# YamaneKoyo/mri-to-speech

Measured on AMD Instinct MI355X. Metric: rtMRI frames/s end-to-end (256x256 frames -> 64-bin mel -> 11413 Hz wav), higher is better.
Workload: dtype bf16x3; 1 GPU; e2e rtMRI->wav, 64 clips x 30 frames per GPU at 256x256 (configs[3] per-GPU share); clips_per_gpu=64, frames_per_clip=30, global_batch_clips=64, hw=256, parallelism=dp1, chunk=1920

## Files before the change

mri-to-speech_amd/csrc/er_sp_fused.hip:

```cpp
#include <algorithm>

#include "kernels.hpp"
#include "prof.hpp"

namespace m2s {
namespace {

__device__ __attribute__((aligned(16))) uint4 g_ersp_zero[4];

__device__ __forceinline__ void dma16(const void* src, void* lds_wave_base) {
  __builtin_amdgcn_global_load_lds(src, lds_wave_base, 16, 0, 0);
}
__device__ __forceinline__ uint32_t lds_off(const void* p) {
  return (uint32_t)(size_t)(const __attribute__((address_space(3))) char*)p;
}
__device__ __forceinline__ uint2 lds_u2(const void* p) {
  uint2 r;
  asm volatile("ds_read_b64 %0, %1\n\ts_waitcnt lgkmcnt(0)" : "=v"(r) : "v"(lds_off(p)));
  return r;
}
__device__ __forceinline__ float4 lds_f4(const void* p) {
  float4 r;
  asm volatile("ds_read_b128 %0, %1\n\ts_waitcnt lgkmcnt(0)" : "=v"(r) : "v"(lds_off(p)));
  return r;
}
template <int N>
__device__ __forceinline__ void wait_vm() {
  asm volatile("s_waitcnt vmcnt(%0)" ::"n"(N) : "memory");
}
__device__ __forceinline__ bf16x8 frag(const char* p) { return *reinterpret_cast<const bf16x8*>(p); }
__device__ __forceinline__ f32x4 mfma(bf16x8 a, bf16x8 b, f32x4 c) {
  return __builtin_amdgcn_mfma_f32_16x16x32_bf16(a, b, c, 0, 0, 0);
}

struct ErSpArgs {
  const bf16_t* x;
  const bf16_t* wst;
  const float* bexp;
  const float* bpwl;
  bf16_t* y;
  int N, H, W, tiles_x, tiles_y;
};

template <int TH, int CSI, int NT, int ON, int NW, int MRG>
__global__ void __launch_bounds__(64 * NW, NW == 4 ? 2 : 1) er_sp_kernel(const ErSpArgs a) {
  constexpr int TW = 16, HW = TW + 2, HH = TH + 2, HPIX = HH * HW;
  constexpr int HPB = (HPIX + 63) / 64;
  constexpr int HPLANE = HPB * 1024;
  constexpr int CH = CSI / 8;
  constexpr int HBUF = 2 * CH * HPLANE;
  constexpr int HP = 2 * CH * HPB / NW;
  static_assert((2 * CH * HPB) % NW == 0, "halo pieces must divide over the waves");
  constexpr int PPW = (MRG * NT + NW - 1) / NW;
  constexpr int SLOT = PPW * NW * 1024;
  constexpr int KC = CSI / 32, NCE = 9 * KC * 2;
  constexpr int MID = NT * 16, KS = MID / 32, PN = ON * KS;
  constexpr int NPS = (PN + NT - 1) / NT;
  constexpr int NST = (NCE + 2 * NPS) / MRG;
  static_assert(MRG == 1 || (MRG == 2 && NPS == 1 && NCE % 2 == 0), "merged stages");
  constexpr int RPW = TH / NW;
  constexpr int ST = RPW * ON * 2;
  static_assert(NT % 2 == 0 && ON * 16 == CSI && TH % NW == 0, "er_sp shape");

  extern __shared__ __attribute__((aligned(16))) char smem[];
  char* ring = smem;
  char* hbuf = smem + 3 * SLOT;
  float* bexp_l = reinterpret_cast<float*>(hbuf + 2 * HBUF);
  const int tid = threadIdx.x, lane = tid & 63;
  const int wave = __builtin_amdgcn_readfirstlane(tid >> 6);
  const int g = lane >> 4, r16 = lane & 15;
  const int tpi = a.tiles_x * a.tiles_y, ntiles = a.N * tpi;

  const void* zpage = g_ersp_zero;
  asm volatile("" : "+s"(zpage));
  auto stage_dma = [&](int ls, int slot) {
#pragma unroll
    for (int j = 0; j < PPW; ++j) {
      const int piece = wave * PPW + j;
      const void* src = piece < MRG * NT ? (const void*)(a.wst + ((size_t)(ls * MRG * NT + piece) * 64 + lane) * 8) : zpage;
      dma16(src, ring + slot * SLOT + piece * 1024);
    }
  };
  auto halo_dma = [&](int tile, char* buf) {
    const int n = tile / tpi, tr = tile - n * tpi;
    const int ty0 = (tr / a.tiles_x) * TH - 1, tx0 = (tr - (tr / a.tiles_x) * a.tiles_x) * TW - 1;
    const bf16_t* xi = a.x + (size_t)n * a.H * a.W * (2 * CSI);
#pragma unroll
    for (int j = 0; j < HP; ++j) {
      const int piece = wave * HP + j, pc = piece / HPB, pb = piece - pc * HPB;
      const int p = pb * 64 + lane, hy = p / HW, hx = p - hy * HW;
      const int iy = ty0 + hy, ix = tx0 + hx;
      const void* src = zpage;
      if (p < HPIX && iy >= 0 && iy < a.H && ix >= 0 && ix < a.W)
        src = xi + ((size_t)iy * a.W + ix) * (2 * CSI) + (pc / CH) * CSI + (pc % CH) * 8;
      dma16(src, buf + pc * HPLANE + pb * 1024);
    }
  };

  for (int i = tid; i < MID; i += 64 * NW) bexp_l[i] = a.bexp[i];
  __syncthreads();
  float4 bp[ON];
#pragma unroll
  for (int on = 0; on < ON; ++on) bp[on] = *reinterpret_cast<const float4*>(a.bpwl + on * 16 + 4 * g);

#ifndef ERSP_PRIO
#define ERSP_PRIO 1
#endif
  if (ERSP_PRIO && NW == 8 && wave >= 4) __builtin_amdgcn_s_setprio(1);
  int q = 0;
  if ((int)blockIdx.x < ntiles) {
    stage_dma(0, 0);
    stage_dma(1, 1);
    halo_dma(blockIdx.x, hbuf);
  }
  for (int it = 0, tile = blockIdx.x; tile < ntiles; tile += gridDim.x, ++it) {
    const bool has_next = tile + (int)gridDim.x < ntiles;
    const char* hb = hbuf + (it & 1) * HBUF;
    const int n = tile / tpi, tr = tile - n * tpi;
    const int oy0 = (tr / a.tiles_x) * TH, ox = (tr - (tr / a.tiles_x) * a.tiles_x) * TW + r16;

    auto begin_stage = [&](int ls) -> const char* {
      if (ls == 0) {
        if (it == 0) wait_vm<0>();
        else wait_vm<PPW + ST>();
      } else if (ls == 1) {
        if (has_next) wait_vm<ST + PPW + HP>();
        else wait_vm<ST + PPW>();
      } else if (ls == 2) {
        if (has_next) wait_vm<HP + PPW>();
        else wait_vm<PPW>();
      } else if (ls + 1 < NST || has_next) {
        wait_vm<PPW>();
      } else {
        wait_vm<0>();
      }
      __builtin_amdgcn_s_barrier();
      asm volatile("" ::: "memory");
      if (ls + 2 < NST) stage_dma(ls + 2, (q + 2) % 3);
      else if (has_next) stage_dma(ls + 2 - NST, (q + 2) % 3);
      if (ls == 0 && has_next) halo_dma(tile + gridDim.x, hbuf + ((it + 1) & 1) * HBUF);
      const char* ws = ring + (q % 3) * SLOT + lane * 16;
      ++q;
      return ws;
    };

    f32x4 acc[RPW][NT];
#pragma unroll
    for (int i = 0; i < RPW; ++i)
#pragma unroll
      for (int nt = 0; nt < NT; ++nt) acc[i][nt] = f32x4{0.f, 0.f, 0.f, 0.f};
#pragma unroll 1
    for (int ks = 0; ks < 9 * KC; ++ks) {
      const int t = ks / KC, kc = ks - t * KC, ky = t / 3, kx = t - (t / 3) * 3;
      bf16x8 bh[RPW], bl[RPW];
      const char* wsm = MRG == 2 ? begin_stage(ks) : nullptr;
      {
        const char* ws = MRG == 2 ? wsm : begin_stage(2 * ks);
#pragma unroll
        for (int i = 0; i < RPW; ++i) {
          const int pix = (RPW * wave + i + ky) * HW + r16 + kx;
          bh[i] = frag(hb + (kc * 4 + g) * HPLANE + pix * 16);
          bl[i] = frag(hb + (CH + kc * 4 + g) * HPLANE + pix * 16);
        }
#pragma unroll
        for (int nt = 0; nt < NT; ++nt) {
          const bf16x8 af = frag(ws + nt * 1024);
#pragma unroll
          for (int i = 0; i < RPW; ++i) acc[i][nt] = mfma(af, bl[i], mfma(af, bh[i], acc[i][nt]));
        }
      }
      {
        const char* ws = MRG == 2 ? wsm + NT * 1024 : begin_stage(2 * ks + 1);
#pragma unroll
        for (int nt = 0; nt < NT; ++nt) {
          const bf16x8 af = frag(ws + nt * 1024);
#pragma unroll
          for (int i = 0; i < RPW; ++i) acc[i][nt] = mfma(af, bh[i], acc[i][nt]);
        }
      }
    }

    bf16x8 mh[RPW][KS], ml[RPW][KS];
#pragma unroll
    for (int kk = 0; kk < KS; ++kk)
#pragma unroll
      for (int i = 0; i < RPW; ++i) {
        float v[8];
#pragma unroll
        for (int hh = 0; hh < 2; ++hh) {
          const int nt = 2 * kk + hh;
          const float4 bb = lds_f4(bexp_l + nt * 16 + 4 * g);
          v[4 * hh + 0] = silu(acc[i][nt][0] + bb.x);
          v[4 * hh + 1] = silu(acc[i][nt][1] + bb.y);
          v[4 * hh + 2] = silu(acc[i][nt][2] + bb.z);
          v[4 * hh + 3] = silu(acc[i][nt][3] + bb.w);
// ... 7 lines not shown

    f32x4 o[RPW][ON];
#pragma unroll
    for (int i = 0; i < RPW; ++i)
#pragma unroll
      for (int on = 0; on < ON; ++on) o[i][on] = f32x4{0.f, 0.f, 0.f, 0.f};
    const char* wpm = MRG == 2 ? begin_stage(NCE / 2) : nullptr;
#pragma unroll
    for (int pl = 0; pl < 2; ++pl)
#pragma unroll
      for (int ps = 0; ps < NPS; ++ps) {
        const char* ws = MRG == 2 ? wpm + pl * NT * 1024 : begin_stage(NCE + pl * NPS + ps);
#pragma unroll
        for (int nt = 0; nt < NT; ++nt) {
          const int j = ps * NT + nt;
          if (j >= PN) break;
          const int kk = j / ON, on = j - (j / ON) * ON;
          const bf16x8 af = frag(ws + nt * 1024);
#pragma unroll
          for (int i = 0; i < RPW; ++i) {
            o[i][on] = mfma(af, mh[i][kk], o[i][on]);
            if (pl == 0) o[i][on] = mfma(af, ml[i][kk], o[i][on]);
          }
        }
      }

#pragma unroll
    for (int i = 0; i < RPW; ++i) {
      const int ry = RPW * wave + i, oy = oy0 + ry;
      const int cpix = ((ry + 1) * HW + r16 + 1) * 16;
#pragma unroll
      for (int on = 0; on < ON; ++on) {
        const int c4 = on * 16 + 4 * g;
        float rh[4], rl[4];
        unpack_bf16x4(lds_u2(hb + (c4 >> 3) * HPLANE + cpix + (c4 & 7) * 2), rh);
        unpack_bf16x4(lds_u2(hb + (CH + (c4 >> 3)) * HPLANE + cpix + (c4 & 7) * 2), rl);
        const float v[4] = {o[i][on][0] + bp[on].x + rh[0] + rl[0], o[i][on][1] + bp[on].y + rh[1] + rl[1],
                            o[i][on][2] + bp[on].z + rh[2] + rl[2], o[i][on][3] + bp[on].w + rh[3] + rl[3]};
        uint2 h, l;
        split4(v, h, l);
        bf16_t* yo = a.y + (((size_t)n * a.H + oy) * a.W + ox) * (2 * CSI) + c4;
        *reinterpret_cast<uint2*>(yo) = h;
        *reinterpret_cast<uint2*>(yo + CSI) = l;
      }
    }
  }
  wait_vm<0>();
}

template <int TH, int CSI, int NT, int ON, int NW, int MRG>
void launch_t(const ErSpArgs& a, const char* name, double flops, double bytes, hipStream_t s) {
  constexpr int HW = 18, HPB = ((TH + 2) * HW + 63) / 64, CH = CSI / 8, PPW = (MRG * NT + NW - 1) / NW;
  const size_t lds = 3 * (size_t)PPW * NW * 1024 + 2 * (size_t)(2 * CH * HPB * 1024) + NT * 16 * sizeof(float);
  M2S_CHECK(lds <= (NW == 4 ? 80 : 160) * 1024, "er_sp: LDS budget");
  allow_lds(reinterpret_cast<const void*>(&er_sp_kernel<TH, CSI, NT, ON, NW, MRG>));
  const int cus = device_cus();
  const int grid = std::min(a.N * a.tiles_x * a.tiles_y, (NW == 4 ? 2 : 1) * cus);
  ProfScope ps(name, flops, bytes, s);
  hipLaunchKernelGGL((er_sp_kernel<TH, CSI, NT, ON, NW, MRG>), dim3(grid), dim3(64 * NW), lds, s, a);
  M2S_HIP(hipGetLastError());
}

int tile_rows(int cs_in) { return cs_in == 32 ? 16 : 8; }

}

bool er_sp_supported(int H, int W, int cs_in, int mid, int cs_out) {
  const bool shape = (cs_in == 32 && mid == 128 && cs_out == 32) || (cs_in == 64 && mid == 224 && cs_out == 64);
  return shape && H > 0 && W > 0 && W % 16 == 0 && H % tile_rows(cs_in) == 0;
}

int er_sp_nt_stages(int cs_in, int mid, int cs_out, int* nt) {
  *nt = mid / 16;
  const int kc = cs_in / 32, pn = (cs_out / 16) * (mid / 32);
  return 9 * kc * 2 + 2 * ((pn + *nt - 1) / *nt);
}

void launch_er_sp(const void* x, int N, int H, int W, int cs_in, int mid, int cs_out, const void* wst, const float* bexp,
                  const float* bpwl, void* y, double flops, double bytes, hipStream_t s, bool merged) {
  M2S_CHECK(er_sp_supported(H, W, cs_in, mid, cs_out) && N > 0, "er_sp: unsupported shape");
  ErSpArgs a;
  a.x = static_cast<const bf16_t*>(x);
  a.wst = static_cast<const bf16_t*>(wst);
  a.bexp = bexp;
  a.bpwl = bpwl;
  a.y = static_cast<bf16_t*>(y);
  a.N = N;
  a.H = H;
  a.W = W;
  a.tiles_x = W / 16;
  a.tiles_y = H / tile_rows(cs_in);
  if (cs_in == 32 && merged)
    launch_t<16, 32, 8, 2, 8, 2>(a, "er_sp_kernel<16, 32, 8, 2, 8, 2>", flops, bytes, s);
  else if (cs_in == 32)
    launch_t<16, 32, 8, 2, 8, 1>(a, "er_sp_kernel<16, 32, 8, 2, 8, 1>", flops, bytes, s);
  else
    launch_t<8, 64, 14, 4, 8, 1>(a, "er_sp_kernel<8, 64, 14, 4, 8, 1>", flops, bytes, s);
}

}
```

mri-to-speech_amd/csrc/kernels.hpp:

```cpp
#pragma once

#include "m2s_common.hpp"

namespace m2s {

enum AsyncCode : unsigned { M2S_ASYNC_LSTM = 1u, M2S_ASYNC_WS = 2u };
struct AsyncReport {
  unsigned spin_max = 1u << 20;
  unsigned* err = nullptr;
};
__device__ __forceinline__ void report_async(unsigned* err, unsigned code, int lane) {
  if (err && lane == 0) __hip_atomic_store(err, code, __ATOMIC_RELAXED, __HIP_MEMORY_SCOPE_SYSTEM);
}

template <typename T>
void launch_stem(const float* frames, int N, int H, int W, int OH, int OW, int pad_t, int pad_l,
                 const float* w9, const float* bias, int cout, int cs_out, T* y, hipStream_t s);

int dw_pixel_blocks(int OH, int OW);
template <typename T>
void launch_dwconv(const T* x, int N, int IH, int IW, int OH, int OW, int stride, int pad_t, int pad_l,
                   int C, int cs, const float* w9, const float* bias, T* y, float* sums, hipStream_t s);

template <typename T>
// ... 50 lines not shown
void launch_rb1_fused(const bf16_t* x, bf16_t* s, int B, int L, int C, int k, int np, const int* dil,
                      const bf16_t* const* w1, const float* const* b1, const bf16_t* const* w2,
                      const float* const* b2, int kp, int accum, float div, bool split, double flops, double bytes,
                      hipStream_t st);

void launch_stem_b0(const float* frames, int N, int H, int W, int OH, int OW, int pad_t, int pad_l, const float* w9,
                    const float* b9, const void* w0, const float* b0, int kp0, const void* w1, const float* b1,
                    int kp1, void* y, bool split, double flops, double bytes, hipStream_t s);

bool se_excite_supported(int rd, int kp2, int cs_mid);
void launch_se_excite(const void* mean, int N, int mid, int cs_mid, const void* w1, int kp1, const float* b1,
                      int rd, const void* w2, int kp2, const float* b2, void* gate, bool split, hipStream_t s);

bool er_fused_supported(int H, int W, int cin, int mid, int cout, int kp_exp, int kp_pwl);
void launch_er_fused(const bf16_t* x, int N, int H, int W, const bf16_t* wexp, const float* bexp, const bf16_t* wpwl,
                     const float* bpwl, bf16_t* y, double flops, double bytes, hipStream_t s);

bool er8_fused_supported(int H, int W, int cin, int mid, int cout);
void launch_er8_fused(const bf16_t* x, int N, int H, int W, const uint8_t* wexp, const float* sexp, const float* bexp,
                      const uint8_t* wpwl, const float* spwl, const float* bpwl, bf16_t* y, double flops, double bytes,
                      hipStream_t s, const uint8_t* x8 = nullptr, uint8_t* y8 = nullptr);

bool er2_fused_supported(int H, int W, int cs_in, int mid, int cout, int kp_exp, int kp_pwl);
int er2_stage_elems();
bool er8w_fused_supported(int H, int W, int cs_in, int mid, int cout);
size_t er8w_stream_bytes();
void launch_er8w_fused(const bf16_t* x, const uint8_t* x8, int N, int H, int W, const uint8_t* wst, const float* sexp,
                       const float* bexp, const float* spwl, const float* bpwl, bf16_t* y, uint8_t* y8, double flops,
                       double bytes, hipStream_t s);
void launch_er2_fused(const bf16_t* x, int N, int H, int W, const bf16_t* wst, const float* bexp, const float* bpwl,
                      bf16_t* y, double flops, double bytes, hipStream_t s);

bool er_sp_supported(int H, int W, int cs_in, int mid, int cs_out);
int er_sp_nt_stages(int cs_in, int mid, int cs_out, int* nt);
void launch_er_sp(const void* x, int N, int H, int W, int cs_in, int mid, int cs_out, const void* wst, const float* bexp,
                  const float* bpwl, void* y, double flops, double bytes, hipStream_t s, bool merged = true);

bool ers2_fused_supported(int OH, int OW, int cs_in, int mid, int cs_out, int kp_exp, int kp_pwl);
int ers2_exp_elems(int cs_in, int mid);
bool ers2_sp_supported(int OH, int OW, int cs_in, int mid, int cs_out);
void launch_ers2_sp(const void* x, int N, int H, int W, int OH, int OW, int pad_t, int pad_l, int cs_in, int mid,
                    int cs_out, const void* wexp, const float* bexp, const void* wpwl, const float* bpwl, void* y,
                    double flops, double bytes, hipStream_t s);
void launch_ers2_fused(const bf16_t* x, int N, int H, int W, int OH, int OW, int pad_t, int pad_l, int cs_in, int mid,
                       int cs_out, const bf16_t* wexp, const float* bexp, const bf16_t* wpwl, const float* bpwl,
                       bf16_t* y, double flops, double bytes, hipStream_t s, uint8_t* y8 = nullptr);

void launch_preprocess(const uint8_t* frames, int N, int H, int W, int channels, float* out, hipStream_t s);

template <typename T>
void launch_gap(const T* x, int N, int P, int C, int cs, float* feats, hipStream_t s);

void launch_lstm_step(const float* pre, const float* whh, float* hs, float* cst, int B, int T, int H,
                      int step, hipStream_t s);

bool lstm_persistent_supported(int H);
size_t lstm_persistent_sync_bytes();
bool lstm_small_supported(int B, int H);
size_t lstm_small_sync_bytes();
void launch_lstm_small(const float* pre, const float* whh, float* hs, int B, int T, int H, void* sync, unsigned spin_max,
                       unsigned* err_host, hipStream_t s, unsigned* epoch = nullptr);
constexpr unsigned LSTM_SPIN_MAX = 1u << 24;
bool lstm_mid_supported(int B, int H);
size_t lstm_mid_sync_bytes();
void launch_lstm_mid(const float* pre, const float* whh, float* hs, int B, int T, int H, void* sync, unsigned spin_max,
                     unsigned* err_host, hipStream_t s);
void launch_lstm_persistent(const float* pre, const float* whh, float* hs, int B, int T, int H, void* sync,
                            unsigned spin_max, unsigned* err_host, hipStream_t s);
bool lstm_x3g_supported(int B, int H);
// ... 60 lines not shown
```

mri-to-speech_amd/csrc/model.cpp:

```cpp
#include "model.hpp"

#include <algorithm>
#include <cmath>
#include <cstdlib>
#include <cstring>
#include <type_traits>

#include "pack.hpp"
#include "prof.hpp"

namespace m2s {

StateDict make_state_dict(const m2s_tensor* t, int n) {
  StateDict sd;
  for (int i = 0; i < n; ++i) {
    M2S_CHECK(t[i].name != nullptr, "state dict entry without a name");
    if (t[i].elem != M2S_ELEM_F32) continue;
    M2S_CHECK(t[i].ndim >= 0 && t[i].ndim <= 4, std::string("bad ndim for ") + t[i].name);
    HostTensor h;
    h.data = static_cast<const float*>(t[i].data);
    for (int d = 0; d < t[i].ndim; ++d) h.shape.push_back(t[i].shape[d]);
    sd[t[i].name] = h;
  }
  return sd;
// ... 31 lines not shown
  BN r;
  r.a.resize(c);
  r.b.resize(c);
  for (int i = 0; i < c; ++i) {
    const float invstd = 1.0f / std::sqrt(v[i] + 1e-3f);
    r.a[i] = invstd * w[i];
    r.b[i] = bb[i] - m[i] * r.a[i];
  }
  return r;
}

Acoustic::Acoustic(const StateDict& sd, int n_mels, int hidden, int dtype, int device)
    : dtype_(dtype), device_(device), n_mels_(n_mels), hidden_(hidden) {
  M2S_CHECK(dtype == M2S_DT_F32 || dtype == M2S_DT_BF16 || dtype == M2S_DT_BF16X3 || dtype == M2S_DT_FP8, "bad dtype");
  M2S_CHECK(n_mels > 0 && hidden > 0 && hidden % 8 == 0, "bad n_mels / rnn_hidden");
  if (const char* e = std::getenv("M2S_IR_FUSED")) ir_fused_ = std::strcmp(e, "0") != 0;
  if (const char* e = std::getenv("M2S_IR_WS")) ir_ws_ = std::strcmp(e, "0") != 0;
  if (const char* e = std::getenv("M2S_IR_WS_S2")) ir_ws_s2_ = std::strcmp(e, "0") != 0;
  if (const char* e = std::getenv("M2S_IRWS_MIN")) irws_min_ = std::atoi(e);
  if (const char* e = std::getenv("M2S_IRWS_F32")) irws_f32_ = std::strcmp(e, "0") != 0;
  if (const char* e = std::getenv("M2S_SEWS_MIN")) sews_min_cus_ = std::atoi(e);
  if (const char* e = std::getenv("M2S_STEM_FUSED")) stem_fused_ = std::strcmp(e, "0") != 0;
  if (const char* e = std::getenv("M2S_F8_EXPAND")) f8_expand_ = std::strcmp(e, "0") != 0;
  if (const char* e = std::getenv("M2S_F8_S2")) f8_s2_ = std::strcmp(e, "0") != 0;
  if (const char* e = std::getenv("M2S_F8_ER")) f8_er_ = std::strcmp(e, "0") != 0;
  if (const char* e = std::getenv("M2S_ER8_X8")) er8_x8_ = std::strcmp(e, "0") != 0;
  if (const char* e = std::getenv("M2S_F8_ER2")) f8_er2_ = std::strcmp(e, "0") != 0;
  if (const char* e = std::getenv("M2S_SE_Y8")) se_y8_ = std::strcmp(e, "0") != 0;
  if (const char* e = std::getenv("M2S_SE_FUSED")) se_fused_ = std::strcmp(e, "0") != 0;
  if (const char* e = std::getenv("M2S_ER_FUSED")) er_fused_ = std::strcmp(e, "0") != 0;
  if (const char* e = std::getenv("M2S_SE_SP")) se_sp_ = std::strcmp(e, "0") != 0;
  if (const char* e = std::getenv("M2S_SE_WS")) se_ws_ = std::strcmp(e, "0") != 0;
  if (const char* e = std::getenv("M2S_ER_MRG")) er_mrg_ = std::strcmp(e, "0") != 0;
  if (const char* e = std::getenv("M2S_IR_S2BAND")) ir_s2band_ = std::strcmp(e, "0") != 0;
  if (const char* e = std::getenv("M2S_LSTM_PERSISTENT")) lstm_persistent_ = std::strcmp(e, "0") != 0;
  if (const char* e = std::getenv("M2S_LSTM_MID")) lstm_mid_ = std::strcmp(e, "0") != 0;
  if (const char* e = std::getenv("M2S_LSTM_X3")) lstm_x3_ = std::strcmp(e, "0") != 0;
  if (const char* e = std::getenv("M2S_LSTM_X3G")) lstm_x3g_ = std::strcmp(e, "0") != 0;
  const std::string P = "cnn.backbone.";
  {
    const float* w = need(sd, P + "conv_stem.weight", {EFF_STEM, 3, 3, 3}).data;
    BN bn = fold_bn(sd, P + "bn1", EFF_STEM);
    std::vector<float> w9(EFF_STEM * 9);
    for (int o = 0; o < EFF_STEM; ++o)
      for (int t = 0; t < 9; ++t)
        w9[o * 9 + t] = (w[(o * 3 + 0) * 9 + t] + w[(o * 3 + 1) * 9 + t] + w[(o * 3 + 2) * 9 + t]) * bn.a[o];
    stem_w_ = arena_.add_vec(w9);
    stem_b_ = arena_.add_vec(bn.b);
  }
  const int pdt = dtype == M2S_DT_FP8 ? M2S_DT_BF16 : dtype;
  int cin = EFF_STEM;
  for (int s = 0; s < 6; ++s) {
    const StageDef& sdf = kStages[s];
    for (int r = 0; r < sdf.reps; ++r) {
      Block b;
      b.type = sdf.type;
      b.stride = r == 0 ? sdf.stride : 1;
      b.cin = cin;
      b.cout = sdf.cout;
      b.skip = b.stride == 1 && cin == sdf.cout;
      const std::string q = P + "blocks." + std::to_string(s) + "." + std::to_string(r) + ".";
      const int k = sdf.k;
      auto conv2d_kxk = [&](PConv& pc, const std::string& wk, int ci, int co, const BN& bn) {
        const float* w = need(sd, wk, {co, ci, k, k}).data;
        pc = make_pconv(KIND_CONV2D, ci, co, k * k, pdt);
        pc.ks = k;
        pc.stride = b.stride;
        pc.macs_per_row = (double)co * ci * k * k;
        pack_conv(arena_, pdt, pc, [&](int, int n, int t, int c) { return w[((size_t)n * ci + c) * k * k + t] * bn.a[n]; },
                  [&](int n) { return bn.b[n]; });
      };
      auto conv1x1 = [&](PConv& pc, const std::string& wk, int ci, int co, const BN& bn) {
        const float* w = need(sd, wk, {co, ci, 1, 1}).data;
        pc = make_pconv(KIND_GEMM, ci, co, 1, pdt);
        pc.macs_per_row = (double)co * ci;
        pack_conv(arena_, pdt, pc, [&](int, int n, int, int c) { return w[(size_t)n * ci + c] * bn.a[n]; },
                  [&](int n) { return bn.b[n]; });
      };
      if (b.type == 0) {
        conv2d_kxk(b.c1, q + "conv.weight", cin, b.cout, fold_bn(sd, q + "bn1", b.cout));
      } else if (b.type == 1) {
        b.mid = make_divisible(cin * (double)sdf.exp);
        conv2d_kxk(b.c1, q + "conv_exp.weight", cin, b.mid, fold_bn(sd, q + "bn1", b.mid));
        conv1x1(b.c2, q + "conv_pwl.weight", b.mid, b.cout, fold_bn(sd, q + "bn2", b.cout));
        if (dtype == M2S_DT_BF16X3 && b.stride == 1 && b.skip && k == 3 &&
            er_sp_supported(32, 32, b.c1.cs_in, b.mid, chan_stride(b.cout))) {
          int nt = 0;
          const int csi = b.c1.cs_in, cso = chan_stride(b.cout), nst = er_sp_nt_stages(csi, b.mid, cso, &nt);
          const int kc = csi / 32, nce = 9 * kc * 2, on_n = cso / 16, pn = on_n * (b.mid / 32), nps = (pn + nt - 1) / nt;
          const float* we = need(sd, q + "conv_exp.weight", {b.mid, cin, 3, 3}).data;
          const float* wq = need(sd, q + "conv_pwl.weight", {b.cout, b.mid, 1, 1}).data;
          const BN e1 = fold_bn(sd, q + "bn1", b.mid), e2 = fold_bn(sd, q + "bn2", b.cout);
          std::vector<uint16_t> st((size_t)nst * nt * 64 * 8, 0);
          for (int sg = 0; sg < nst; ++sg)
            for (int pc = 0; pc < nt; ++pc)
              for (int ln = 0; ln < 64; ++ln)
                for (int e = 0; e < 8; ++e) {
                  const int row = ln & 15, g8 = ln >> 4;
                  float v = 0.f;
                  int plane;
                  if (sg < nce) {
                    plane = sg & 1;
                    const int ks = sg >> 1, t = ks / kc, c = (ks % kc) * 32 + 8 * g8 + e, n = 16 * pc + row;
                    if (c < cin) v = we[((size_t)n * cin + c) * 9 + t] * e1.a[n];
                  } else {
                    plane = (sg - nce) / nps;
                    const int j = ((sg - nce) % nps) * nt + pc;
                    if (j >= pn) continue;
                    const int kk = j / on_n, on = j % on_n, o = on * 16 + row;
                    const int c = 32 * kk + (e < 4 ? 4 * g8 + e : 16 + 4 * g8 + e - 4);
                    if (o < b.cout) v = wq[(size_t)o * b.mid + c] * e2.a[o];
                  }
                  uint16_t hi, lo;
                  split_host(v, &hi, &lo);
                  st[(((size_t)sg * nt + pc) * 64 + ln) * 8 + e] = plane == 0 ? hi : lo;
                }
          b.er_sp_w = arena_.add_vec(st);
          b.er_sp = true;
        } else if (dtype == M2S_DT_BF16X3 && b.stride == 2 && k == 3 &&
                   ers2_sp_supported(8, 16, b.c1.cs_in, b.mid, chan_stride(b.cout))) {
          const int csi = b.c1.cs_in, cso = chan_stride(b.cout), ks_n = (9 * csi + 31) / 32, ntn = b.mid / 16;
          const int onn = cso / 16, pkn = b.mid / 32;
          const float* we = need(sd, q + "conv_exp.weight", {b.mid, cin, 3, 3}).data;
          const float* wq = need(sd, q + "conv_pwl.weight", {b.cout, b.mid, 1, 1}).data;
          const BN e1 = fold_bn(sd, q + "bn1", b.mid), e2 = fold_bn(sd, q + "bn2", b.cout);
          const size_t fe_half = (size_t)ks_n * ntn * 64 * 8, fp_half = (size_t)onn * pkn * 64 * 8;
          std::vector<uint16_t> fe(2 * fe_half, 0), fp(2 * fp_half, 0);
          for (int s2 = 0; s2 < ks_n; ++s2)
            for (int nt = 0; nt < ntn; ++nt)
              for (int ln = 0; ln < 64; ++ln)
                for (int e = 0; e < 8; ++e) {
                  const int g8 = ln >> 4, n = nt * 16 + (ln & 15), t = 2 * s2 + (g8 >> 1), c = 8 * (g8 & 1) + e;
                  const float v = t < 9 && c < cin ? we[((size_t)n * cin + c) * 9 + t] * e1.a[n] : 0.f;
                  const size_t i = (((size_t)s2 * ntn + nt) * 64 + ln) * 8 + e;
                  split_host(v, &fe[i], &fe[fe_half + i]);
                }
          for (int on = 0; on < onn; ++on)
            for (int ks = 0; ks < pkn; ++ks)
              for (int ln = 0; ln < 64; ++ln)
                for (int e = 0; e < 8; ++e) {
                  const int n = on * 16 + (ln & 15), g4 = 4 * (ln >> 4);
                  const int c = 32 * ks + (e < 4 ? g4 + e : 16 + g4 + e - 4);
                  const float v = n < b.cout ? wq[(size_t)n * b.mid + c] * e2.a[n] : 0.f;
                  const size_t i = (((size_t)on * pkn + ks) * 64 + ln) * 8 + e;
                  split_host(v, &fp[i], &fp[fp_half + i]);
                }
          b.er_wexp = arena_.add_vec(fe);
          b.er_wpwl = arena_.add_vec(fp);
          b.ers_sp = true;
        } else if (pdt == M2S_DT_BF16 && b.stride == 1 && b.skip && k == 3 &&
            er_fused_supported(64, 64, cin, b.mid, b.cout, b.c1.kp, b.c2.kp)) {
// ... 369 lines not shown
  a.IW = p.ow;
  a.OH = p.nh;
  a.OW = p.nw;
  a.pad_t = p.qt;
  a.pad_l = p.ql;
  a.M = p.nc * p.nh * p.nw;
  return a;
}

template <typename T>
void Acoustic::effnet_cn(EffPass<T>& p, size_t k) {
  const Block& b = blocks_[k];
  ConvArgs a = conv2d_args(p, b.c1, p.cur, p.nxt);
  a.act = ACT_SILU;
  a.res = b.skip ? p.cur : nullptr;
  run_conv<T>(a, b.c1, p.s);
}

template <typename T>
void Acoustic::effnet_er(EffPass<T>& p, size_t k) {
  const Block& b = blocks_[k];
  const int nc = p.nc, oh = p.oh, ow = p.ow, nh = p.nh, nw = p.nw, qt = p.qt, ql = p.ql;
  T *const cur = p.cur, *const nxt = p.nxt, *const M = p.b.M;
  uint8_t *const cur8 = p.cur8, *const *const X8 = p.b.X8, *&next8 = p.next8;
  hipStream_t s = p.s;
  const double px = (double)nc * nh * nw;
  uint8_t* const er8_next = X8[0] && f8_er_ && k + 1 < blocks_.size() &&
                                    ((er8_x8_ && blocks_[k + 1].er8) || (f8_er2_ && blocks_[k + 1].er8w))
                                ? (cur8 == X8[0] ? X8[1] : X8[0])
                                : nullptr;
  if (std::is_same<T, sp_t>::value && er_fused_ && b.er_sp &&
      er_sp_supported(nh, nw, b.c1.cs_in, b.mid, chan_stride(b.cout))) {
    launch_er_sp(cur, nc, nh, nw, b.c1.cs_in, b.mid, chan_stride(b.cout), arena_.ptr(b.er_sp_w), b.c1.b, b.c2.b, nxt,
                 2.0 * px * b.mid * (9.0 * b.cin + b.cout), 4.0 * px * (b.c1.cs_in + chan_stride(b.cout)), s, er_mrg_);
  } else if (std::is_same<T, sp_t>::value && er_fused_ && b.ers_sp && b.stride == 2 &&
             ers2_sp_supported(nh, nw, b.c1.cs_in, b.mid, chan_stride(b.cout))) {
    launch_ers2_sp(cur, nc, oh, ow, nh, nw, qt, ql, b.c1.cs_in, b.mid, chan_stride(b.cout), arena_.ptr(b.er_wexp),
                   b.c1.b, arena_.ptr(b.er_wpwl), b.c2.b, nxt, 2.0 * px * b.mid * (9.0 * b.cin + b.cout),
                   4.0 * ((double)nc * oh * ow * b.c1.cs_in + px * chan_stride(b.cout)), s);
  } else if (std::is_same<T, bf16_t>::value && er_fused_ && f8_er_ && b.er8 &&
             er8_fused_supported(nh, nw, b.cin, b.mid, b.cout)) {
    uint8_t* y8 = cur8 && er8_next && er8_fused_supported(nh, nw, b.cout, b.mid, b.cout) ? er8_next : nullptr;
    launch_er8_fused(reinterpret_cast<const bf16_t*>(cur), nc, nh, nw, static_cast<const uint8_t*>(arena_.ptr(b.er8_wexp)),
                     static_cast<const float*>(arena_.ptr(b.er8_sexp)), b.c1.b,
                     static_cast<const uint8_t*>(arena_.ptr(b.er8_wpwl)), static_cast<const float*>(arena_.ptr(b.er8_spwl)),
                     b.c2.b, reinterpret_cast<bf16_t*>(nxt), 2.0 * px * b.mid * (9.0 * b.cin + b.cout),
                     2.0 * px * (2.0 * b.cin) + (3.0 * 8 * 2048 + 2 * 2048), s, cur8, y8);
    next8 = y8;
  } else if (std::is_same<T, bf16_t>::value && er_fused_ && b.er_frag &&
             er_fused_supported(nh, nw, b.cin, b.mid, b.cout, b.c1.kp, b.c2.kp)) {
    launch_er_fused(reinterpret_cast<const bf16_t*>(cur), nc, nh, nw,
                    static_cast<const bf16_t*>(arena_.ptr(b.er_wexp)), b.c1.b,
                    static_cast<const bf16_t*>(arena_.ptr(b.er_wpwl)), b.c2.b, reinterpret_cast<bf16_t*>(nxt),
                    2.0 * px * b.mid * (9.0 * b.cin + b.cout), 2.0 * px * (2.0 * b.cin) + 2.0 * (9.0 * 32 * 128 + 128 * 32), s);
  } else if (std::is_same<T, bf16_t>::value && er_fused_ && f8_er_ && f8_er2_ && b.er8w && cur8 &&
             er8w_fused_supported(nh, nw, b.c1.cs_in, b.mid, b.cout)) {
    uint8_t* y8 = er8_next && blocks_[k + 1].er8w ? er8_next : nullptr;
    launch_er8w_fused(reinterpret_cast<const bf16_t*>(cur), cur8, nc, nh, nw, static_cast<const uint8_t*>(arena_.ptr(b.er8w_w)),
                      static_cast<const float*>(arena_.ptr(b.er8w_sexp)), b.c1.b,
                      static_cast<const float*>(arena_.ptr(b.er8w_spwl)), b.c2.b, reinterpret_cast<bf16_t*>(nxt), y8,
                      2.0 * px * b.mid * (9.0 * b.cin + b.cout),
                      px * (b.cin + 2.0 * b.cin + 2.0 * b.cout + (y8 ? b.cout : 0.0)) + (9.0 * b.cin + b.cout) * b.mid, s);
    next8 = y8;
  } else if (std::is_same<T, bf16_t>::value && er_fused_ && b.er_frag &&
             er2_fused_supported(nh, nw, b.c1.cs_in, b.mid, b.cout, b.c1.kp, b.c2.kp)) {
    launch_er2_fused(reinterpret_cast<const bf16_t*>(cur), nc, nh, nw, static_cast<const bf16_t*>(arena_.ptr(b.er_wexp)),
                     b.c1.b, b.c2.b, reinterpret_cast<bf16_t*>(nxt), 2.0 * px * b.mid * (9.0 * b.cin + b.cout),
// ... 1322 lines not shown
```

mri-to-speech_amd/csrc/model.hpp:

```cpp
#pragma once

#include <map>
#include <string>
#include <vector>

#include "../../include/m2s.h"
#include "conv_igemm.hpp"
#include "kernels.hpp"

namespace m2s {

struct HostTensor {
  const float* data = nullptr;
  std::vector<int64_t> shape;
  size_t numel() const {
    size_t n = 1;
    for (auto d : shape) n *= (size_t)d;
    return n;
  }
};
using StateDict = std::map<std::string, HostTensor>;
StateDict make_state_dict(const m2s_tensor* t, int n);

class Arena {
// ... 105 lines not shown
  ~Acoustic();
  Acoustic(const Acoustic&) = delete;
  Acoustic& operator=(const Acoustic&) = delete;
  unsigned take_async_error();
  unsigned lstm_spin_max_ = LSTM_SPIN_MAX;
  unsigned ws_spin_max_ = 1u << 20;
  AsyncReport ws_report() const {
    AsyncReport r;
    r.spin_max = ws_spin_max_;
    r.err = err_dev_;
    return r;
  }
  int device() const { return device_; }
  int n_mels() const { return n_mels_; }
  int chunk = 1920;
  bool ir_fused_ = true;
  bool ir_ws_ = true;
  bool ir_ws_s2_ = true;
  int irws_min_ = 512;
  bool irws_f32_ = true;
  int sews_min_cus_ = 1;
  bool stem_fused_ = true;
  bool f8_er_ = true;
  bool se_y8_ = true;
  bool f8_er2_ = true;
  bool er8_x8_ = true;
  bool f8_expand_ = true;
  bool f8_s2_ = true;
  bool se_fused_ = true;
  bool er_fused_ = true;
  bool se_sp_ = false;
  bool se_ws_ = true;
  bool er_mrg_ = true;
  bool ir_s2band_ = true;
  bool lstm_persistent_ = true;
  bool lstm_mid_ = true;
  bool lstm_x3_ = true;
  bool lstm_x3g_ = true;

  size_t workspace_bytes(int B, int T, int H, int W) const;
  void forward(const float* frames, int B, int T, int H, int W, float* mel_norm, Workspace& ws, hipStream_t s);
  void effnet(const float* frames, int N, int H, int W, float* feats, int stop_after, float* probe, int* probe_dims,
              Workspace& ws, hipStream_t s);
  void bilstm(const float* feats, int B, int T, float* y, float* mel_norm, Workspace& ws, hipStream_t s);
  size_t ragged_workspace_bytes(const int* lengths, int B, int H, int W) const;
  void bilstm_ragged(const float* feats, const int* lengths, int B, long N, float* y, float* mel_norm, Workspace& ws,
                     hipStream_t s);
  void forward_ragged(const float* frames, const int* lengths, int B, long N, int H, int W, float* mel_norm,
                      Workspace& ws, hipStream_t s);
  size_t windowed_workspace_bytes(const int* lengths, const int* context, int B, int H, int W, int window,
                                  int merge) const;
  void bilstm_windowed(const float* feats, const int* lengths, const int* context, int B, long N, int window, int merge,
                       float* y, float* mel_norm, Workspace& ws, hipStream_t s);
  void forward_windowed(const float* frames, const int* lengths, const int* context, int B, long N, int H, int W,
                        int window, int merge, float* mel_norm, Workspace& ws, hipStream_t s);

 private:
  struct WindowBufs {
    int* tab = nullptr;
    int2* win = nullptr;
    float *pre = nullptr, *c = nullptr, *hm = nullptr, *hf = nullptr;
    void* hop[2] = {nullptr, nullptr};
  };
  WindowBufs window_bufs(Workspace& ws, const WindowPlan& p) const;
  template <typename T>
  struct EffBufs {
// ... 16 lines not shown
    LstmBufs d;
  };
  RaggedLstmBufs ragged_lstm_bufs(Workspace& ws, const RaggedDims& d) const;
  template <typename T>
  struct EffPass {
    EffBufs<T> b;
    hipStream_t s;
    int nc, n0, oh, ow, nh, nw, qt, ql;
    T *cur, *nxt;
    uint8_t *cur8, *next8;
    bool f8, sews, mid_f32;
  };
  size_t whh_win_ = 0;
  void lstm_recurrence(const float* pre, float* hs, float* cst, void* sync, int B, int T, double seq_steps, double rows,
                       hipStream_t s);
  static size_t lstm_sync_bytes();
  RaggedTable rtab_;
  struct Block {
    int type = 0;
    int stride = 1, cin = 0, cout = 0, mid = 0, rd = 0;
    bool skip = false;
    PConv c1, c2;
    size_t dw_w = 0, dw_b = 0;
    size_t dw_w2 = 0;
    PConv se1, se2;
    size_t er_wexp = 0, er_wpwl = 0;
    bool er_frag = false;
    size_t er8_wexp = 0, er8_sexp = 0, er8_wpwl = 0, er8_spwl = 0;
    bool er8 = false;
    size_t er8w_w = 0, er8w_sexp = 0, er8w_spwl = 0;
    bool er8w = false;
    size_t er_sp_w = 0;
    bool er_sp = false;
    bool ers_sp = false;
    size_t f8_w = 0, f8_s = 0, f8_b = 0;
    int f8_kp = 0, f8_npad = 0;
    bool f8_pwl = false;
    size_t f8x_w = 0, f8x_s = 0;
    int f8x_kp = 0;
    bool f8_pw = false;
  };
  template <typename T>
  void effnet_t(const float* frames, int N, int H, int W, float* feats, int stop_after, float* probe, int* probe_dims,
                Workspace& ws, hipStream_t s);
  template <typename T>
  void effnet_cn(EffPass<T>& p, size_t k);
  template <typename T>
  void effnet_er(EffPass<T>& p, size_t k);
  template <typename T>
  void effnet_ir_front(EffPass<T>& p, size_t k);
  template <typename T>
  void effnet_ir_se(EffPass<T>& p, size_t k);
  template <typename T>
  void effnet_ir_pwl(EffPass<T>& p, size_t k);
  int pass_frames(int N) const;
  size_t effnet_x8(int H, int W) const;
  void effnet_dims(int H, int W, size_t* io_elems, size_t* mid_elems, size_t* se_elems) const;

  int dtype_, device_, n_mels_, hidden_;
  Arena arena_;
  size_t stem_w_ = 0, stem_b_ = 0;
  std::vector<Block> blocks_;
  PConv lstm_ih_;
  size_t whh_ = 0, head_wt_ = 0, head_b_ = 0;
  int max_mid_cs_ = 0;
  unsigned* err_host_ = nullptr;
// ... 118 lines not shown
```

Before: 50490 rtMRI frames/s.

## Add stride-2 variant of fused edge-residual kernel and optional packed-K path

```diff
diff --git a/mri-to-speech_amd/csrc/er_sp_fused.hip b/mri-to-speech_amd/csrc/er_sp_fused.hip
--- a/mri-to-speech_amd/csrc/er_sp_fused.hip
+++ b/mri-to-speech_amd/csrc/er_sp_fused.hip
@@ -40,32 +40,41 @@
   const float* bpwl;
   bf16_t* y;
   int N, H, W, tiles_x, tiles_y;
+  int OH, OW, pad_t, pad_l;
 };
 
-template <int TH, int CSI, int NT, int ON, int NW, int MRG>
+template <int TH, int CSI, int NT, int ON, int NW, int MRG, int CR, int S>
 __global__ void __launch_bounds__(64 * NW, NW == 4 ? 2 : 1) er_sp_kernel(const ErSpArgs a) {
-  constexpr int TW = 16, HW = TW + 2, HH = TH + 2, HPIX = HH * HW;
+  constexpr int TW = 16, HW = S == 2 ? TW + 1 : TW + 2, HH = S == 2 ? 2 * TH + 1 : TH + 2, HPIX = HH * HW;
   constexpr int HPB = (HPIX + 63) / 64;
   constexpr int HPLANE = HPB * 1024;
   constexpr int CH = CSI / 8;
-  constexpr int HBUF = 2 * CH * HPLANE;
-  constexpr int HP = 2 * CH * HPB / NW;
-  static_assert((2 * CH * HPB) % NW == 0, "halo pieces must divide over the waves");
+  constexpr int NPL = 2 * CH * S;
+  constexpr int HBUF = NPL * HPLANE;
+  constexpr int NHB = S == 2 ? 1 : 2;
+  constexpr int HP = NPL * HPB / NW;
+  static_assert((NPL * HPB) % NW == 0, "halo pieces must divide over the waves");
   constexpr int PPW = (MRG * NT + NW - 1) / NW;
   constexpr int SLOT = PPW * NW * 1024;
-  constexpr int KC = CSI / 32, NCE = 9 * KC * 2;
+  constexpr bool KPACK = CR < CH;
+  constexpr int KC = CSI / 32, NKS = KPACK ? (9 * CR + 3) / 4 : 9 * KC;
+  constexpr int NCE = NKS * 2;
+  static_assert(CR >= 1 && CR <= CH, "er_sp real chunks");
   constexpr int MID = NT * 16, KS = MID / 32, PN = ON * KS;
   constexpr int NPS = (PN + NT - 1) / NT;
   constexpr int NST = (NCE + 2 * NPS) / MRG;
   static_assert(MRG == 1 || (MRG == 2 && NPS == 1 && NCE % 2 == 0), "merged stages");
   constexpr int RPW = TH / NW;
   constexpr int ST = RPW * ON * 2;
-  static_assert(NT % 2 == 0 && ON * 16 == CSI && TH % NW == 0, "er_sp shape");
+  constexpr int CSO = ON * 16;
+  constexpr int HST = S == 2 ? NCE : 0;
+  static_assert(NT % 2 == 0 && TH % NW == 0 && (S == 1 ? CSO == CSI : S == 2), "er_sp shape");
+  static_assert(S == 1 || (!KPACK && MRG == 1 && HST >= 3 && HST + 2 < NST - 1), "er_sp stride 2");
 
   extern __shared__ __attribute__((aligned(16))) char smem[];
   char* ring = smem;
   char* hbuf = smem + 3 * SLOT;
-  float* bexp_l = reinterpret_cast<float*>(hbuf + 2 * HBUF);
+  float* bexp_l = reinterpret_cast<float*>(hbuf + NHB * HBUF);
   const int tid = threadIdx.x, lane = tid & 63;
   const int wave = __builtin_amdgcn_readfirstlane(tid >> 6);
   const int g = lane >> 4, r16 = lane & 15;
@@ -82,18 +91,19 @@
     }
   };
   auto halo_dma = [&](int tile, char* buf) {
-    const int n = tile / tpi, tr = tile - n * tpi;
-    const int ty0 = (tr / a.tiles_x) * TH - 1, tx0 = (tr - (tr / a.tiles_x) * a.tiles_x) * TW - 1;
+    const int n = tile / tpi, tr = tile - n * tpi, ty = tr / a.tiles_x, tx = tr - ty * a.tiles_x;
+    const int ty0 = S == 2 ? 2 * TH * ty - a.pad_t : ty * TH - 1, tx0 = S == 2 ? 2 * TW * tx - a.pad_l : tx * TW - 1;
     const bf16_t* xi = a.x + (size_t)n * a.H * a.W * (2 * CSI);
 #pragma unroll
     for (int j = 0; j < HP; ++j) {
-      const int piece = wave * HP + j, pc = piece / HPB, pb = piece - pc * HPB;
-      const int p = pb * 64 + lane, hy = p / HW, hx = p - hy * HW;
+      const int piece = wave * HP + j, pl = piece / HPB, pb = piece - pl * HPB;
+      const int pc = pl / S, par = pl - pc * S;
+      const int p = pb * 64 + lane, hy = p / HW, hs = p - hy * HW, hx = S == 2 ? 2 * hs + par : hs;
       const int iy = ty0 + hy, ix = tx0 + hx;
       const void* src = zpage;
-      if (p < HPIX && iy >= 0 && iy < a.H && ix >= 0 && ix < a.W)
+      if (p < HPIX && (S == 1 || hx <= 2 * TW) && iy >= 0 && iy < a.H && ix >= 0 && ix < a.W && pc % CH < CR)
         src = xi + ((size_t)iy * a.W + ix) * (2 * CSI) + (pc / CH) * CSI + (pc % CH) * 8;
-      dma16(src, buf + pc * HPLANE + pb * 1024);
+      dma16(src, buf + pl * HPLANE + pb * 1024);
     }
   };
 
@@ -115,7 +125,7 @@
   }
   for (int it = 0, tile = blockIdx.x; tile < ntiles; tile += gridDim.x, ++it) {
     const bool has_next = tile + (int)gridDim.x < ntiles;
-    const char* hb = hbuf + (it & 1) * HBUF;
+    const char* hb = hbuf + (it & (NHB - 1)) * HBUF;
     const int n = tile / tpi, tr = tile - n * tpi;
     const int oy0 = (tr / a.tiles_x) * TH, ox = (tr - (tr / a.tiles_x) * a.tiles_x) * TW + r16;
 
@@ -123,6 +133,13 @@
       if (ls == 0) {
         if (it == 0) wait_vm<0>();
         else wait_vm<PPW + ST>();
+      } else if (S == 2 && ls == 1) {
+        wait_vm<ST + PPW>();
+      } else if (S == 2 && ls == 2) {
+        wait_vm<PPW>();
+      } else if (S == 2 && (ls == HST + 1 || ls == HST + 2)) {
+        if (has_next) wait_vm<PPW + HP>();
+        else wait_vm<PPW>();
       } else if (ls == 1) {
         if (has_next) wait_vm<ST + PPW + HP>();
         else wait_vm<ST + PPW>();
@@ -138,7 +155,7 @@
       asm volatile("" ::: "memory");
       if (ls + 2 < NST) stage_dma(ls + 2, (q + 2) % 3);
       else if (has_next) stage_dma(ls + 2 - NST, (q + 2) % 3);
-      if (ls == 0 && has_next) halo_dma(tile + gridDim.x, hbuf + ((it + 1) & 1) * HBUF);
+      if (ls == HST && has_next) halo_dma(tile + gridDim.x, hbuf + ((it + 1) & (NHB - 1)) * HBUF);
       const char* ws = ring + (q % 3) * SLOT + lane * 16;
       ++q;
       return ws;
@@ -150,17 +167,20 @@
 #pragma unroll
       for (int nt = 0; nt < NT; ++nt) acc[i][nt] = f32x4{0.f, 0.f, 0.f, 0.f};
 #pragma unroll 1
-    for (int ks = 0; ks < 9 * KC; ++ks) {
-      const int t = ks / KC, kc = ks - t * KC, ky = t / 3, kx = t - (t / 3) * 3;
+    for (int ks = 0; ks < NKS; ++ks) {
+      const int f = KPACK ? min(4 * ks + g, 9 * CR - 1) : 0;
+      const int t = KPACK ? f / CR : ks / KC, kc = ks - t * KC, ky = t / 3, kx = t - (t / 3) * 3;
+      const int cpl = S == 2 ? (kc * 4 + g) * 2 + (kx & 1) : KPACK ? f - t * CR : kc * 4 + g;
+      const int kxs = S == 2 ? kx >> 1 : kx;
       bf16x8 bh[RPW], bl[RPW];
       const char* wsm = MRG == 2 ? begin_stage(ks) : nullptr;
       {
         const char* ws = MRG == 2 ? wsm : begin_stage(2 * ks);
 #pragma unroll
         for (int i = 0; i < RPW; ++i) {
-          const int pix = (RPW * wave + i + ky) * HW + r16 + kx;
-          bh[i] = frag(hb + (kc * 4 + g) * HPLANE + pix * 16);
-          bl[i] = frag(hb + (CH + kc * 4 + g) * HPLANE + pix * 16);
+          const int pix = (S * (RPW * wave + i) + ky) * HW + r16 + kxs;
+          bh[i] = frag(hb + cpl * HPLANE + pix * 16);
+          bl[i] = frag(hb + (CH * S + cpl) * HPLANE + pix * 16);
         }
 #pragma unroll
         for (int nt = 0; nt < NT; ++nt) {
@@ -234,32 +254,35 @@
 #pragma unroll
       for (int on = 0; on < ON; ++on) {
         const int c4 = on * 16 + 4 * g;
-        float rh[4], rl[4];
-        unpack_bf16x4(lds_u2(hb + (c4 >> 3) * HPLANE + cpix + (c4 & 7) * 2), rh);
-        unpack_bf16x4(lds_u2(hb + (CH + (c4 >> 3)) * HPLANE + cpix + (c4 & 7) * 2), rl);
+        float rh[4] = {0.f, 0.f, 0.f, 0.f}, rl[4] = {0.f, 0.f, 0.f, 0.f};
+        if (S == 1) {
+          unpack_bf16x4(lds_u2(hb + (c4 >> 3) * HPLANE + cpix + (c4 & 7) * 2), rh);
+          unpack_bf16x4(lds_u2(hb + (CH + (c4 >> 3)) * HPLANE + cpix + (c4 & 7) * 2), rl);
+        }
         const float v[4] = {o[i][on][0] + bp[on].x + rh[0] + rl[0], o[i][on][1] + bp[on].y + rh[1] + rl[1],
                             o[i][on][2] + bp[on].z + rh[2] + rl[2], o[i][on][3] + bp[on].w + rh[3] + rl[3]};
         uint2 h, l;
         split4(v, h, l);
-        bf16_t* yo = a.y + (((size_t)n * a.H + oy) * a.W + ox) * (2 * CSI) + c4;
+        bf16_t* yo = a.y + (((size_t)n * (S == 2 ? a.OH : a.H) + oy) * (S == 2 ? a.OW : a.W) + ox) * (2 * CSO) + c4;
         *reinterpret_cast<uint2*>(yo) = h;
-        *reinterpret_cast<uint2*>(yo + CSI) = l;
+        *reinterpret_cast<uint2*>(yo + CSO) = l;
       }
     }
   }
   wait_vm<0>();
 }
 
-template <int TH, int CSI, int NT, int ON, int NW, int MRG>
+template <int TH, int CSI, int NT, int ON, int NW, int MRG, int CR, int S = 1>
 void launch_t(const ErSpArgs& a, const char* name, double flops, double bytes, hipStream_t s) {
-  constexpr int HW = 18, HPB = ((TH + 2) * HW + 63) / 64, CH = CSI / 8, PPW = (MRG * NT + NW - 1) / NW;
-  const size_t lds = 3 * (size_t)PPW * NW * 1024 + 2 * (size_t)(2 * CH * HPB * 1024) + NT * 16 * sizeof(float);
+  constexpr int HPIX = S == 2 ? (2 * TH + 1) * 17 : (TH + 2) * 18, HPB = (HPIX + 63) / 64, CH = CSI / 8;
+  constexpr int PPW = (MRG * NT + NW - 1) / NW, NHB = S == 2 ? 1 : 2;
+  const size_t lds = 3 * (size_t)PPW * NW * 1024 + NHB * (size_t)(2 * CH * S * HPB * 1024) + NT * 16 * sizeof(float);
   M2S_CHECK(lds <= (NW == 4 ? 80 : 160) * 1024, "er_sp: LDS budget");
-  allow_lds(reinterpret_cast<const void*>(&er_sp_kernel<TH, CSI, NT, ON, NW, MRG>));
+  allow_lds(reinterpret_cast<const void*>(&er_sp_kernel<TH, CSI, NT, ON, NW, MRG, CR, S>));
   const int cus = device_cus();
   const int grid = std::min(a.N * a.tiles_x * a.tiles_y, (NW == 4 ? 2 : 1) * cus);
   ProfScope ps(name, flops, bytes, s);
-  hipLaunchKernelGGL((er_sp_kernel<TH, CSI, NT, ON, NW, MRG>), dim3(grid), dim3(64 * NW), lds, s, a);
+  hipLaunchKernelGGL((er_sp_kernel<TH, CSI, NT, ON, NW, MRG, CR, S>), dim3(grid), dim3(64 * NW), lds, s, a);
   M2S_HIP(hipGetLastError());
 }
 
@@ -272,15 +295,49 @@
   return shape && H > 0 && W > 0 && W % 16 == 0 && H % tile_rows(cs_in) == 0;
 }
 
-int er_sp_nt_stages(int cs_in, int mid, int cs_out, int* nt) {
+int er_sp_kpack_chunks(int cs_in, int cin) { return cs_in == 64 && cin == 56 ? 7 : 0; }
+
+int er_sp_nt_stages(int cs_in, int mid, int cs_out, int* nt, int cr) {
   *nt = mid / 16;
-  const int kc = cs_in / 32, pn = (cs_out / 16) * (mid / 32);
-  return 9 * kc * 2 + 2 * ((pn + *nt - 1) / *nt);
+  const int nks = cr ? (9 * cr + 3) / 4 : 9 * (cs_in / 32), pn = (cs_out / 16) * (mid / 32);
+  return nks * 2 + 2 * ((pn + *nt - 1) / *nt);
 }
 
 void launch_er_sp(const void* x, int N, int H, int W, int cs_in, int mid, int cs_out, const void* wst, const float* bexp,
-                  const float* bpwl, void* y, double flops, double bytes, hipStream_t s, bool merged) {
+                  const float* bpwl, void* y, double flops, double bytes, hipStream_t s, bool merged, int cr) {
   M2S_CHECK(er_sp_supported(H, W, cs_in, mid, cs_out) && N > 0, "er_sp: unsupported shape");
+  M2S_CHECK(cr == 0 || (cs_in == 64 && cr == 7), "er_sp: no packed-K kernel for this shape");
+  ErSpArgs a;
+  a.x = static_cast<const bf16_t*>(x);
+  a.wst = static_cast<const bf16_t*>(wst);
+  a.bexp = bexp;
+  a.bpwl = bpwl;
+  a.y = static_cast<bf16_t*>(y);
+  a.N = N;
+  a.H = a.OH = H;
+  a.W = a.OW = W;
+  a.pad_t = a.pad_l = 0;
+  a.tiles_x = W / 16;
+  a.tiles_y = H / tile_rows(cs_in);
+  if (cs_in == 32 && merged)
+    launch_t<16, 32, 8, 2, 8, 2, 4>(a, "er_sp_kernel<16, 32, 8, 2, 8, 2, 4, 1>", flops, bytes, s);
+  else if (cs_in == 32)
+    launch_t<16, 32, 8, 2, 8, 1, 4>(a, "er_sp_kernel<16, 32, 8, 2, 8, 1, 4, 1>", flops, bytes, s);
+  else if (cr == 7)
+    launch_t<8, 64, 14, 4, 8, 1, 7>(a, "er_sp_kernel<8, 64, 14, 4, 8, 1, 7, 1>", flops, bytes, s);
+  else
+    launch_t<8, 64, 14, 4, 8, 1, 8>(a, "er_sp_kernel<8, 64, 14, 4, 8, 1, 8, 1>", flops, bytes, s);
+}
+
+bool er_sp_s2_supported(int OH, int OW, int cs_in, int mid, int cs_out) {
+  return cs_in == 32 && mid == 128 && cs_out == 64 && OH > 0 && OW > 0 && OH % 4 == 0 && OW % 16 == 0;
+}
+
+void launch_er_sp_s2(const void* x, int N, int H, int W, int OH, int OW, int pad_t, int pad_l, int cs_in, int mid,
+                     int cs_out, const void* wst, const float* bexp, const float* bpwl, void* y, double flops,
+                     double bytes, hipStream_t s) {
+  M2S_CHECK(er_sp_s2_supported(OH, OW, cs_in, mid, cs_out) && N > 0, "er_sp stride 2: unsupported shape");
+  M2S_CHECK(pad_t >= 0 && pad_l >= 0 && pad_t <= 1 && pad_l <= 1 && H > 0 && W > 0, "er_sp stride 2: pads");
   ErSpArgs a;
   a.x = static_cast<const bf16_t*>(x);
   a.wst = static_cast<const bf16_t*>(wst);
@@ -290,14 +347,13 @@
   a.N = N;
   a.H = H;
   a.W = W;
-  a.tiles_x = W / 16;
-  a.tiles_y = H / tile_rows(cs_in);
-  if (cs_in == 32 && merged)
-    launch_t<16, 32, 8, 2, 8, 2>(a, "er_sp_kernel<16, 32, 8, 2, 8, 2>", flops, bytes, s);
-  else if (cs_in == 32)
-    launch_t<16, 32, 8, 2, 8, 1>(a, "er_sp_kernel<16, 32, 8, 2, 8, 1>", flops, bytes, s);
-  else
-    launch_t<8, 64, 14, 4, 8, 1>(a, "er_sp_kernel<8, 64, 14, 4, 8, 1>", flops, bytes, s);
-}
-
-}
+  a.OH = OH;
+  a.OW = OW;
+  a.pad_t = pad_t;
+  a.pad_l = pad_l;
+  a.tiles_x = OW / 16;
+  a.tiles_y = OH / 4;
+  launch_t<4, 32, 8, 4, 4, 1, 4, 2>(a, "er_sp_kernel<4, 32, 8, 4, 4, 1, 4, 2>", flops, bytes, s);
+}
+
+}
diff --git a/mri-to-speech_amd/csrc/kernels.hpp b/mri-to-speech_amd/csrc/kernels.hpp
--- a/mri-to-speech_amd/csrc/kernels.hpp
+++ b/mri-to-speech_amd/csrc/kernels.hpp
@@ -106,9 +106,15 @@
                       bf16_t* y, double flops, double bytes, hipStream_t s);
 
 bool er_sp_supported(int H, int W, int cs_in, int mid, int cs_out);
-int er_sp_nt_stages(int cs_in, int mid, int cs_out, int* nt);
+int er_sp_kpack_chunks(int cs_in, int cin);
+int er_sp_nt_stages(int cs_in, int mid, int cs_out, int* nt, int cr = 0);
 void launch_er_sp(const void* x, int N, int H, int W, int cs_in, int mid, int cs_out, const void* wst, const float* bexp,
-                  const float* bpwl, void* y, double flops, double bytes, hipStream_t s, bool merged = true);
+                  const float* bpwl, void* y, double flops, double bytes, hipStream_t s, bool merged = true, int cr = 0);
+
+bool er_sp_s2_supported(int OH, int OW, int cs_in, int mid, int cs_out);
+void launch_er_sp_s2(const void* x, int N, int H, int W, int OH, int OW, int pad_t, int pad_l, int cs_in, int mid,
+                     int cs_out, const void* wst, const float* bexp, const float* bpwl, void* y, double flops,
+                     double bytes, hipStream_t s);
 
 bool ers2_fused_supported(int OH, int OW, int cs_in, int mid, int cs_out, int kp_exp, int kp_pwl);
 int ers2_exp_elems(int cs_in, int mid);
diff --git a/mri-to-speech_amd/csrc/model.cpp b/mri-to-speech_amd/csrc/model.cpp
--- a/mri-to-speech_amd/csrc/model.cpp
+++ b/mri-to-speech_amd/csrc/model.cpp
@@ -87,6 +87,8 @@
   if (const char* e = std::getenv("M2S_SE_SP")) se_sp_ = std::strcmp(e, "0") != 0;
   if (const char* e = std::getenv("M2S_SE_WS")) se_ws_ = std::strcmp(e, "0") != 0;
   if (const char* e = std::getenv("M2S_ER_MRG")) er_mrg_ = std::strcmp(e, "0") != 0;
+  if (const char* e = std::getenv("M2S_ERS2_B20")) ers2_b20_ = std::strcmp(e, "0") != 0;
+  if (const char* e = std::getenv("M2S_ER_KPACK")) er_kpack_ = std::strcmp(e, "0") != 0;
   if (const char* e = std::getenv("M2S_IR_S2BAND")) ir_s2band_ = std::strcmp(e, "0") != 0;
   if (const char* e = std::getenv("M2S_LSTM_PERSISTENT")) lstm_persistent_ = std::strcmp(e, "0") != 0;
   if (const char* e = std::getenv("M2S_LSTM_MID")) lstm_mid_ = std::strcmp(e, "0") != 0;
@@ -138,11 +140,13 @@
         b.mid = make_divisible(cin * (double)sdf.exp);
         conv2d_kxk(b.c1, q + "conv_exp.weight", cin, b.mid, fold_bn(sd, q + "bn1", b.mid));
         conv1x1(b.c2, q + "conv_pwl.weight", b.mid, b.cout, fold_bn(sd, q + "bn2", b.cout));
-        if (dtype == M2S_DT_BF16X3 && b.stride == 1 && b.skip && k == 3 &&
-            er_sp_supported(32, 32, b.c1.cs_in, b.mid, chan_stride(b.cout))) {
+        const bool sp_s1 = b.stride == 1 && b.skip && er_sp_supported(32, 32, b.c1.cs_in, b.mid, chan_stride(b.cout));
+        const bool sp_s2 = ers2_b20_ && b.stride == 2 && er_sp_s2_supported(4, 16, b.c1.cs_in, b.mid, chan_stride(b.cout));
+        if (dtype == M2S_DT_BF16X3 && k == 3 && (sp_s1 || sp_s2)) {
           int nt = 0;
-          const int csi = b.c1.cs_in, cso = chan_stride(b.cout), nst = er_sp_nt_stages(csi, b.mid, cso, &nt);
-          const int kc = csi / 32, nce = 9 * kc * 2, on_n = cso / 16, pn = on_n * (b.mid / 32), nps = (pn + nt - 1) / nt;
+          const int csi = b.c1.cs_in, cso = chan_stride(b.cout), cr = er_kpack_ ? er_sp_kpack_chunks(csi, cin) : 0;
+          const int nst = er_sp_nt_stages(csi, b.mid, cso, &nt, cr);
+          const int on_n = cso / 16, pn = on_n * (b.mid / 32), nps = (pn + nt - 1) / nt, nce = nst - 2 * nps, kc = csi / 32;
           const float* we = need(sd, q + "conv_exp.weight", {b.mid, cin, 3, 3}).data;
           const float* wq = need(sd, q + "conv_pwl.weight", {b.cout, b.mid, 1, 1}).data;
           const BN e1 = fold_bn(sd, q + "bn1", b.mid), e2 = fold_bn(sd, q + "bn2", b.cout);
@@ -156,8 +160,9 @@
                   int plane;
                   if (sg < nce) {
                     plane = sg & 1;
-                    const int ks = sg >> 1, t = ks / kc, c = (ks % kc) * 32 + 8 * g8 + e, n = 16 * pc + row;
-                    if (c < cin) v = we[((size_t)n * cin + c) * 9 + t] * e1.a[n];
+                    const int ks = sg >> 1, f = 4 * ks + g8, n = 16 * pc + row;
+                    const int t = cr ? f / cr : ks / kc, c = cr ? (f % cr) * 8 + e : (ks % kc) * 32 + 8 * g8 + e;
+                    if (t < 9 && c < cin) v = we[((size_t)n * cin + c) * 9 + t] * e1.a[n];
                   } else {
                     plane = (sg - nce) / nps;
                     const int j = ((sg - nce) % nps) * nt + pc;
@@ -171,7 +176,9 @@
                   st[(((size_t)sg * nt + pc) * 64 + ln) * 8 + e] = plane == 0 ? hi : lo;
                 }
           b.er_sp_w = arena_.add_vec(st);
-          b.er_sp = true;
+          b.er_sp = sp_s1;
+          b.er_sp_s2 = sp_s2;
+          b.er_sp_cr = cr;
         } else if (dtype == M2S_DT_BF16X3 && b.stride == 2 && k == 3 &&
                    ers2_sp_supported(8, 16, b.c1.cs_in, b.mid, chan_stride(b.cout))) {
           const int csi = b.c1.cs_in, cso = chan_stride(b.cout), ks_n = (9 * csi + 31) / 32, ntn = b.mid / 16;
@@ -607,7 +614,13 @@
   if (std::is_same<T, sp_t>::value && er_fused_ && b.er_sp &&
       er_sp_supported(nh, nw, b.c1.cs_in, b.mid, chan_stride(b.cout))) {
     launch_er_sp(cur, nc, nh, nw, b.c1.cs_in, b.mid, chan_stride(b.cout), arena_.ptr(b.er_sp_w), b.c1.b, b.c2.b, nxt,
-                 2.0 * px * b.mid * (9.0 * b.cin + b.cout), 4.0 * px * (b.c1.cs_in + chan_stride(b.cout)), s, er_mrg_);
+                 2.0 * px * b.mid * (9.0 * b.cin + b.cout), 4.0 * px * (b.c1.cs_in + chan_stride(b.cout)), s, er_mrg_,
+                 b.er_sp_cr);
+  } else if (std::is_same<T, sp_t>::value && er_fused_ && b.er_sp_s2 && b.stride == 2 &&
+             er_sp_s2_supported(nh, nw, b.c1.cs_in, b.mid, chan_stride(b.cout))) {
+    launch_er_sp_s2(cur, nc, oh, ow, nh, nw, qt, ql, b.c1.cs_in, b.mid, chan_stride(b.cout), arena_.ptr(b.er_sp_w),
+                    b.c1.b, b.c2.b, nxt, 2.0 * px * b.mid * (9.0 * b.cin + b.cout),
+                    4.0 * ((double)nc * oh * ow * b.c1.cs_in + px * chan_stride(b.cout)), s);
   } else if (std::is_same<T, sp_t>::value && er_fused_ && b.ers_sp && b.stride == 2 &&
              ers2_sp_supported(nh, nw, b.c1.cs_in, b.mid, chan_stride(b.cout))) {
     launch_ers2_sp(cur, nc, oh, ow, nh, nw, qt, ql, b.c1.cs_in, b.mid, chan_stride(b.cout), arena_.ptr(b.er_wexp),
diff --git a/mri-to-speech_amd/csrc/model.hpp b/mri-to-speech_amd/csrc/model.hpp
--- a/mri-to-speech_amd/csrc/model.hpp
+++ b/mri-to-speech_amd/csrc/model.hpp
@@ -161,6 +161,8 @@
   bool se_sp_ = false;
   bool se_ws_ = true;
   bool er_mrg_ = true;
+  bool ers2_b20_ = true;
+  bool er_kpack_ = false;
   bool ir_s2band_ = true;
   bool lstm_persistent_ = true;
   bool lstm_mid_ = true;
@@ -243,6 +245,8 @@
     bool er8w = false;
     size_t er_sp_w = 0;
     bool er_sp = false;
+    bool er_sp_s2 = false;
+    int er_sp_cr = 0;
     bool ers_sp = false;
     size_t f8_w = 0, f8_s = 0, f8_b = 0;
     int f8_kp = 0, f8_npad = 0;
```

Result: no change. 50950 rtMRI frames/s, median of 6 (+0.9%).
